# zkonduit/ezkl

Measured on AMD Instinct MI355X. Metric: BN254 G1 MSM pts/s (2^20 points per GPU; NTT 2^22 elems/s in extra), higher is better.
Workload: dtype u32x8 (254-bit modular integer, Montgomery); 1 GPU; configs[1]: standalone 2^20-point BN254 G1 MSM (uniform scalars, try-and-increment bases) + 2^22 scalar-field NTT per GPU; parallelism=points sharded across 1 rank(s); all_gather of 64-B partials + host fold

## Files before the change

ezkl_amd/csrc/msm.hip:

```cpp
#include "common.hpp"
#include <deque>
#include <thread>
#include <chrono>
#include "curve.hpp"
#include "curve29.hpp"
#include "host64.hpp"
#include <string.h>

namespace ezkl {

static constexpr uint32_t MSM_MAX_PART_BITS = 12;
static constexpr uint32_t MSM_SPAN_HEAVY = 16;
static constexpr uint32_t MSM_PART_STAGE = 13312;
static constexpr uint32_t MSM_BINSORT_STAGE = 15360;
static constexpr uint32_t MSM_HEAVY_CHUNK = 256;
static constexpr uint32_t MSM_DIGIT_E = 8;
static constexpr uint32_t MSM_LMIN = 8;
static constexpr uint32_t MSM_MAX_BIG = 64;
static constexpr uint32_t MSM_BIG_BLOCKS = 64;
static constexpr uint32_t MSM_BIG_ROWS = 8;

__device__ __forceinline__ uint32_t msm_part_of(uint32_t bucket, uint32_t NP) { return bucket ? 1u + (bucket & (NP - 1u)) : 0u; }
__device__ __forceinline__ uint32_t msm_lane_len(const uint32_t* offsets, uint32_t nb, uint32_t nlanes, uint32_t lmin) {
    const uint32_t l = (uint32_t)(((uint64_t)offsets[nb] + nlanes - 1) / nlanes);
    return l < lmin ? lmin : l;
}

template <class T> __device__ __forceinline__ T* bshift(T* p, size_t bytes) {
    return reinterpret_cast<T*>(reinterpret_cast<uintptr_t>(p) + bytes);
}
#define BSH(p) p = bshift(p, _bo)
#define BOFF() const size_t _bo = (size_t)blockIdx.z * bstride

struct WinPlan {
    uint32_t W, base, rem;
    __host__ __device__ uint32_t width(uint32_t w) const { return base + (w < rem ? 1u : 0u); }
    __host__ __device__ uint32_t offset(uint32_t w) const { return w * base + (w < rem ? w : rem); }
    __host__ __device__ uint32_t cmax() const { return base + (rem ? 1u : 0u); }
};
struct MsmTable {
    g1a_t* tab = nullptr;
    WinPlan wp{0, 0, 0};
    size_t n = 0;
    hipEvent_t ready = nullptr;
    bool synced = false;
};
struct MsmSlot;
struct MsmUpload;
struct MsmBatch;
struct MsmState;
static MsmState& msm_state();
#define g_tables (msm_state().tables)
#define g_table_stream (msm_state().table_stream)
#define g_slots (msm_state().slots)
#define g_call_slots (msm_state().call_slots)
#define g_call_claimed (msm_state().call_claimed)
#define g_call_finishing (msm_state().call_finishing)
#define g_call_owner (msm_state().call_owner)
#define g_call_order_ev (msm_state().call_order_ev)
#define g_copy_st (msm_state().copy_st)
#define g_tail_pinned (msm_state().tail_pinned)
#define g_tail_pinned_elems (msm_state().tail_pinned_elems)
#define g_open_upload (msm_state().open_upload)
#define g_open_batch (msm_state().open_batch)

static constexpr int MSM_MAX_SLOTS = 16;
static int msm_slots_init() {
    int v = 4;
    if (const char* e = getenv("EZKL_MSM_SLOTS")) {
        const int x = atoi(e);
        if (x >= 1 && x <= MSM_MAX_SLOTS) v = x;
    }
    return v;
}
static const int MSM_SLOTS = msm_slots_init();
struct MsmSlot {
    hipStream_t st = nullptr;
    uint8_t* scratch = nullptr;
    size_t scratch_bytes = 0;
    uint32_t* pinned = nullptr;
    void* pinned_dev = nullptr;
    size_t pinned_msms = 0;
    const fe_t** list_pinned = nullptr;
    hipEvent_t done = nullptr;
    uint32_t bits = 0;
    uint32_t count = 0;
    void* out = nullptr;
    bool busy = false;
};
static constexpr int MSM_CALL_SLOTS = 4;
struct MsmState {
    std::map<const Bases*, MsmTable> tables;
    hipStream_t table_stream = nullptr;
    MsmSlot slots[MSM_MAX_SLOTS];
    MsmSlot call_slots[MSM_CALL_SLOTS];
    bool call_claimed[MSM_CALL_SLOTS] = {false, false, false, false};
    bool call_finishing[MSM_CALL_SLOTS] = {false, false, false, false};
    std::thread::id call_owner[MSM_CALL_SLOTS];
    hipEvent_t call_order_ev = nullptr;
    hipStream_t copy_st = nullptr;
    fe_t* tail_pinned = nullptr;
    size_t tail_pinned_elems = 0;
    MsmUpload* open_upload = nullptr;
    MsmBatch* open_batch = nullptr;
    bool attrs_set = false;
    int acc_blocks_per_cu = 0;
};
static MsmState& msm_state() {
    Ctx* c = ctx();
    if (!c->msm_state) c->msm_state = new MsmState();
    return *static_cast<MsmState*>(c->msm_state);
}


static WinPlan pick_plan(size_t n) {
    WinPlan best{0, 0, 0};
    double best_cost = 0;
    for (uint32_t W = 10; W <= 127; W++) {
        WinPlan p{W, 254 / W, 254 % W};
        if (p.cmax() > 23) continue;
        const double cost = (double)n * W + 4.0 * (double)((size_t)1 << (p.cmax() - 1));
        if (!best.W || cost < best_cost) { best = p; best_cost = cost; }
    }
    return best;
}

__global__ __launch_bounds__(256) void msm_precompute_kernel(const g1a_t* prev, g1a_t* next, size_t n, uint32_t c) {
    size_t i = (size_t)blockIdx.x * blockDim.x + threadIdx.x;
    if (i >= n) return;
    g1a_t p = ld_g1a(prev + i);
    g1x_t a = g1x_from_affine(p);
    for (uint32_t k = 0; k < c; k++) a = g1x_double(a);
    st_g1a(next + i, g1x_to_affine(a));
}

__global__ __launch_bounds__(256) void msm_table_to_r261_kernel(g1a_t* tab, size_t count) {
    size_t i = (size_t)blockIdx.x * blockDim.x + threadIdx.x;
    if (i >= count) return;
    fe_t k;
#pragma unroll
    for (int q = 0; q < 8; q++) k.v[q] = Fq29C::R261_32[q];
    g1a_t p = ld_g1a(tab + i);
    if (g1a_is_id(p)) return;
    p.x = Fq::mul(p.x, k);
    p.y = Fq::mul(p.y, k);
    st_g1a(tab + i, p);
}

__device__ __forceinline__ bool gt_half_r(const fe_t& s) {
    uint32_t d[8], c = 0, br = 0;
#pragma unroll
    for (int i = 0; i < 8; i++) d[i] = addc32(s.v[i], s.v[i], c);
#pragma unroll
    for (int i = 0; i < 8; i++) (void)subb32(d[i], FrP::MOD[i], br);
    return c != 0 || br == 0;
}
__device__ __forceinline__ fe_t msm_canon(const fe_t* scalars, size_t i, uint32_t& neg) {
    fe_t s = Fr::from_mont(ld_fe(scalars + i));
    neg = 0;
    if (gt_half_r(s)) {
        uint32_t br = 0;
#pragma unroll
        for (int k = 0; k < 8; k++) s.v[k] = subb32(FrP::MOD[k], s.v[k], br);
        neg = 1;
    }
    return s;
}
__device__ __forceinline__ uint32_t msm_take_bits(fe_t& s, uint32_t c) {
    const uint32_t d = s.v[0] & ((1u << c) - 1u);
#pragma unroll
    for (int k = 0; k < 7; k++) s.v[k] = __builtin_amdgcn_alignbit(s.v[k + 1], s.v[k], c);
    s.v[7] >>= c;
    return d;
}
template <class F>
__device__ __forceinline__ void msm_foreach_digit(fe_t s, uint32_t neg, const WinPlan& wp, F&& f) {
    uint32_t carry = 0;
    for (uint32_t w = 0; w < wp.W; w++) {
        const uint32_t c = wp.width(w), half = 1u << (c - 1);
        uint32_t raw = msm_take_bits(s, c) + carry;
        if (raw > half) {
            carry = 1;
            if (raw != (1u << c)) f(w, (1u << c) - raw - 1u, neg ^ 1u);
        } else {
            carry = 0;
            if (raw) f(w, raw - 1u, neg);
        }
    }
}

__device__ __forceinline__ bool msm_digit_step(fe_t& s, uint32_t neg, uint32_t c, uint32_t& carry, uint32_t& bucket, uint32_t& sign) {
    const uint32_t half = 1u << (c - 1);
    const uint32_t raw = msm_take_bits(s, c) + carry;
    if (raw > half) {
        carry = 1;
        bucket = (1u << c) - raw - 1u;
        sign = neg ^ 1u;
        return raw != (1u << c);
    }
    carry = 0;
    bucket = raw - 1u;
    sign = neg;
    return raw != 0;
}

__device__ __forceinline__ uint32_t msm_block_scan(uint32_t v, uint32_t* wsum, uint32_t& total) {
    const uint32_t lane = threadIdx.x & 63u, wave = threadIdx.x >> 6, nw = blockDim.x >> 6;
    uint32_t x = v;
#pragma unroll
    for (uint32_t d = 1; d < 64; d <<= 1) {
        const uint32_t y = __shfl_up(x, d, 64);
        if (lane >= d) x += y;
    }
    if (lane == 63) wsum[wave] = x;
    __syncthreads();
    if (wave == 0) {
        uint32_t s = lane < nw ? wsum[lane] : 0u;
#pragma unroll
        for (uint32_t d = 1; d < 16; d <<= 1) {
            const uint32_t y = __shfl_up(s, d, 64);
            if (lane >= d) s += y;
        }
        if (lane < nw) wsum[lane] = s;
    }
    __syncthreads();
    total = wsum[nw - 1];
    const uint32_t r = x + (wave ? wsum[wave - 1] : 0u);
    __syncthreads();
    return r;
}

__global__ __launch_bounds__(256) void msm_hist_kernel(const fe_t* scalars, size_t n, size_t per_block, WinPlan wp,
                                                       uint32_t LB, uint32_t NP, uint32_t* wg_hist, uint32_t* wg_cnt,
                                                       const fe_t* const* scal_list, uint32_t* zero_base, uint32_t zero_words, size_t bstride) {
    BOFF(); BSH(wg_hist); BSH(wg_cnt);
    if (scal_list) scalars = scal_list[blockIdx.z];
    if (zero_base) {
        BSH(zero_base);
        for (uint32_t i = blockIdx.x * 256 + threadIdx.x; i < zero_words; i += gridDim.x * 256) zero_base[i] = 0;
    }
    __shared__ uint32_t lh[(1u << MSM_MAX_PART_BITS) + 1];
    const uint32_t NQ = NP + 1;
    for (uint32_t p = threadIdx.x; p < NQ; p += 256) lh[p] = 0;
    __syncthreads();
    size_t lo = (size_t)blockIdx.x * per_block, hi = lo + per_block < n ? lo + per_block : n;
    for (size_t i0 = lo + threadIdx.x; i0 < hi; i0 += 4 * 256) {
        fe_t s[4];
        uint32_t neg[4], carry[4] = {0, 0, 0, 0};
#pragma unroll
        for (int q = 0; q < 4; q++) {
            const size_t i = i0 + (size_t)q * 256;
            if (i < hi) s[q] = msm_canon(scalars, i, neg[q]);
            else { s[q] = Fr::zero(); neg[q] = 0; }
        }
        for (uint32_t w = 0; w < wp.W; w++) {
            const uint32_t c = wp.width(w);
#pragma unroll
            for (int q = 0; q < 4; q++) {
                uint32_t bucket, sign;
                if (msm_digit_step(s[q], neg[q], c, carry[q], bucket, sign)) atomicAdd(&lh[msm_part_of(bucket, NP)], 1u);
            }
        }
    }
    __syncthreads();
    for (uint32_t p = threadIdx.x; p < NQ; p += 256) {
        wg_hist[(size_t)blockIdx.x * NQ + p] = lh[p];
        wg_cnt[(size_t)blockIdx.x * NQ + p] = lh[p];
    }
}
__global__ __launch_bounds__(1024) void msm_hist_scan_kernel(uint32_t* wg_hist, uint32_t G, uint32_t NP, uint32_t* part_count, size_t bstride) {
    BOFF(); BSH(wg_hist); BSH(part_count);
    __shared__ uint32_t sums[32][33];
    const uint32_t c = threadIdx.x & 31, j = threadIdx.x >> 5;
    const uint32_t p = blockIdx.x * 32 + c;
    const uint32_t chunk = (G + 31) / 32, g0 = j * chunk, g1 = g0 + chunk < G ? g0 + chunk : G;
    uint32_t s = 0;
    if (p < NP)
        for (uint32_t g = g0; g < g1; g++) s += wg_hist[(size_t)g * NP + p];
    sums[j][c] = s;
    __syncthreads();
    if (j == 0) {
        uint32_t run = 0;
        for (uint32_t q = 0; q < 32; q++) {
            uint32_t v = sums[q][c];
            sums[q][c] = run;
            run += v;
        }
        if (p < NP) part_count[p] = run;
    }
    __syncthreads();
    if (p < NP) {
        uint32_t run = sums[j][c];
        for (uint32_t g = g0; g < g1; g++) {
            uint32_t v = wg_hist[(size_t)g * NP + p];
            wg_hist[(size_t)g * NP + p] = run;
            run += v;
        }
    }
}
__device__ __forceinline__ void msm_part_scan_body(const uint32_t* part_count, uint32_t NQ, uint32_t* part_base, uint32_t* big_flag,
                                                   uint32_t* big_list, uint32_t* big_count, uint32_t* sh) {
    const uint32_t t = threadIdx.x;
    constexpr uint32_t PER = 5;
    uint32_t v[PER], sum = 0;
#pragma unroll
    for (uint32_t q = 0; q < PER; q++) {
        const uint32_t i = PER * t + q;
        v[q] = i < NQ ? part_count[i] : 0;
        sum += v[q];
    }
    uint32_t total;
    uint32_t run = msm_block_scan(sum, sh, total) - sum;
#pragma unroll
    for (uint32_t q = 0; q < PER; q++) {
        const uint32_t i = PER * t + q;
        if (i < NQ) part_base[i] = run;
        run += v[q];
    }
    if (t == 1023) part_base[NQ] = total;
#pragma unroll
    for (uint32_t q = 0; q < PER; q++) {
        const uint32_t i = PER * t + q;
        if (i == 0 || i >= NQ) continue;
        uint32_t slot = 0;
        if (v[q] > MSM_BINSORT_STAGE) {
            slot = atomicAdd(big_count, 1u);
            if (slot < MSM_MAX_BIG) big_list[slot] = i - 1;
            slot = slot < MSM_MAX_BIG ? slot + 1 : 0;
        }
        big_flag[i - 1] = slot;
    }
}
__global__ __launch_bounds__(1024) void msm_part_scan_kernel(const uint32_t* part_count, uint32_t NQ, uint32_t* part_base, uint32_t* big_flag,
                                                             uint32_t* big_list, uint32_t* big_count, size_t bstride) {
    BOFF(); BSH(part_count); BSH(part_base); BSH(big_flag); BSH(big_list); BSH(big_count);
    __shared__ uint32_t sh[1024];
    msm_part_scan_body(part_count, NQ, part_base, big_flag, big_list, big_count, sh);
}
__global__ __launch_bounds__(1024) void msm_partition_kernel(const fe_t* scalars, size_t n, size_t per_block, WinPlan wp,
                                                             uint32_t LB, uint32_t NP, size_t base_offset, size_t tab_stride,
                                                             const uint32_t* part_base, const uint32_t* wg_hist, const uint32_t* wg_cnt, uint2* entries,
                                                             uint32_t* vals, const fe_t* const* scal_list, size_t bstride) {
    BOFF(); BSH(part_base); BSH(wg_hist); BSH(wg_cnt); BSH(entries); BSH(vals);
    if (scal_list) scalars = scal_list[blockIdx.z];
    extern __shared__ uint32_t plds[];
    __shared__ uint32_t tsum[1024];
    const uint32_t NQ = NP + 1;
    uint32_t* start = plds;
    uint32_t* cursor = plds + (NQ + 1);
    uint32_t* gbase = plds + 2 * (NQ + 1);
    uint2* stage = reinterpret_cast<uint2*>(plds + 3 * (NQ + 1));
    const uint32_t t = threadIdx.x, T = blockDim.x;
    const uint32_t K = (NQ + T - 1) / T;
    uint32_t loc = 0;
    for (uint32_t q = 0; q < K; q++) {
        const uint32_t p = t * K + q;
        if (p < NQ) loc += wg_cnt[(size_t)blockIdx.x * NQ + p];
    }
    uint32_t total;
    uint32_t run = msm_block_scan(loc, tsum, total) - loc;
    for (uint32_t q = 0; q < K; q++) {
        const uint32_t p = t * K + q;
        if (p < NQ) {
            start[p] = run;
            cursor[p] = run;
            gbase[p] = part_base[p] + wg_hist[(size_t)blockIdx.x * NQ + p];
            run += wg_cnt[(size_t)blockIdx.x * NQ + p];
        }
    }
    __syncthreads();
    const size_t lo = (size_t)blockIdx.x * per_block, hi = lo + per_block < n ? lo + per_block : n;
    const size_t i = lo + t;
    if (i < hi) {
        uint32_t neg;
        fe_t s = msm_canon(scalars, i, neg);
        msm_foreach_digit(s, neg, wp, [&](uint32_t w, uint32_t bucket, uint32_t sign) {
            const uint32_t r = atomicAdd(&cursor[msm_part_of(bucket, NP)], 1u);
            stage[r] = make_uint2((uint32_t)(w * tab_stride + base_offset + i) | (sign << 31), bucket);
        });
    }
    __syncthreads();
    const uint32_t PB = 31 - __clz(NP);
    for (uint32_t idx = t; idx < total; idx += T) {
        const uint2 e = stage[idx];
        const uint32_t p = msm_part_of(e.y, NP);
        const uint32_t slot = gbase[p] + (idx - start[p]);
        if (p) entries[slot] = make_uint2(e.x, e.y >> PB);
        else vals[slot] = e.x;
    }
}
__device__ __forceinline__ uint32_t msm_wave_rank(uint32_t* cnt, uint32_t key) {
    const uint64_t active = __ballot(1);
    const uint32_t first = __builtin_amdgcn_readfirstlane(key);
    if (__ballot(key == first) == active) {
        const uint32_t rank = (uint32_t)__popcll(active & ((1ull << (threadIdx.x & 63u)) - 1ull));
        uint32_t base = 0;
        if (rank == 0) base = atomicAdd(&cnt[first], (uint32_t)__popcll(active));
        return (uint32_t)__builtin_amdgcn_readfirstlane(base) + rank;
    }
    return atomicAdd(&cnt[key], 1u);
}
__device__ __forceinline__ void msm_bins_scan(uint32_t* cnt, uint32_t* tsum, uint32_t nbins, uint32_t p, uint32_t beg, const uint32_t* part_base,
                                              bool emit, uint32_t* offsets, g1x29_t* buckets) {
    const uint32_t t = threadIdx.x;
    uint32_t loc[4], s = 0;
#pragma unroll
    for (int q = 0; q < 4; q++) {
        uint32_t j = t * 4 + q;
        loc[q] = j < nbins ? cnt[j] : 0;
        s += loc[q];
    }
    uint32_t total;
    uint32_t run = msm_block_scan(s, tsum, total) - s;
#pragma unroll
    for (int q = 0; q < 4; q++) {
        uint32_t j = t * 4 + q;
        if (j < nbins) {
            cnt[j] = run;
            if (emit) {
                const bool b0 = (p == 0 && j == 0);
                offsets[(size_t)p * nbins + j] = b0 ? part_base[0] : beg + run;
                if (b0 ? part_base[1] == part_base[0] : loc[q] == 0) st_f29(&buckets[(size_t)p * nbins + j].zz, Fq29::zero());
            }
        }
        run += loc[q];
    }
    __syncthreads();
// ... 10 lines not shown
    __shared__ uint32_t tsum[512];
    extern __shared__ uint32_t stage[];
    if (blockIdx.x >= NP) {
        BSH(big_list); BSH(big_count); BSH(bin_total); BSH(block_off);
        const uint32_t w = blockIdx.x - NP;
        msm_bigsort_count_body(entries, part_base, LB, big_list, big_count, bin_total, block_off, cnt, w % MSM_BIG_BLOCKS, w / MSM_BIG_BLOCKS, MSM_BIG_ROWS);
        return;
    }
    const uint32_t p = blockIdx.x, t = threadIdx.x, nbins = 1u << LB;
    const uint32_t beg = part_base[p + 1], end = part_base[p + 2];
    if (p == NP - 1 && t == 0) offsets[(size_t)NP * nbins] = end;
    if (big_flag[p]) return;
    const bool staged = (end - beg) <= MSM_BINSORT_STAGE;
    for (uint32_t j = t; j < nbins; j += 512) cnt[j] = 0;
    __syncthreads();
    if (staged) {
        constexpr int PER = MSM_BINSORT_STAGE / 512;
        uint2 v[PER];
#pragma unroll
        for (int q = 0; q < PER; q++) {
            const uint32_t e = beg + t + (uint32_t)q * 512u;
            v[q] = e < end ? entries[e] : make_uint2(0u, 0xffffffffu);
        }
#pragma unroll
        for (int q = 0; q < PER; q++)
            if (v[q].y != 0xffffffffu) atomicAdd(&cnt[v[q].y], 1u);
        __syncthreads();
        msm_bins_scan(cnt, tsum, nbins, p, beg, part_base, true, offsets, buckets);
#pragma unroll
        for (int q = 0; q < PER; q++)
            if (v[q].y != 0xffffffffu) stage[atomicAdd(&cnt[v[q].y], 1u)] = v[q].x;
        __syncthreads();
        for (uint32_t i = t; i < end - beg; i += 512) vals[beg + i] = stage[i];
    } else {
        for (uint32_t e = beg + t; e < end; e += 512) (void)msm_wave_rank(cnt, entries[e].y);
        __syncthreads();
        msm_bins_scan(cnt, tsum, nbins, p, beg, part_base, true, offsets, buckets);
        for (uint32_t e = beg + t; e < end; e += 512) {
            const uint2 v = entries[e];
            vals[beg + msm_wave_rank(cnt, v.y)] = v.x;
        }
    }
}
__device__ __forceinline__ void msm_big_slice(uint32_t beg, uint32_t end, uint32_t& s0, uint32_t& s1, uint32_t bx) {
    const uint32_t chunk = (end - beg + MSM_BIG_BLOCKS - 1) / MSM_BIG_BLOCKS;
    s0 = beg + bx * chunk;
    s1 = s0 + chunk < end ? s0 + chunk : end;
    if (s0 > end) s0 = end;
}
__device__ __forceinline__ void msm_bigsort_count_body(const uint2* entries, const uint32_t* part_base, uint32_t LB, const uint32_t* big_list,
                                                       const uint32_t* big_count, uint32_t* bin_total, uint32_t* block_off, uint32_t* cnt, uint32_t bx,
                                                       uint32_t by, uint32_t rows) {
    const uint32_t t = threadIdx.x, nbins = 1u << LB;
    const uint32_t nbig = big_count[0] < MSM_MAX_BIG ? big_count[0] : MSM_MAX_BIG;
    for (uint32_t y = by; y < nbig; y += rows) {
        const uint32_t p = big_list[y];
        uint32_t s0, s1;
        msm_big_slice(part_base[p + 1], part_base[p + 2], s0, s1, bx);
        for (uint32_t j = t; j < nbins; j += 512) cnt[j] = 0;
        __syncthreads();
        for (uint32_t e = s0 + t; e < s1; e += 512) (void)msm_wave_rank(cnt, entries[e].y);
        __syncthreads();
        for (uint32_t j = t; j < nbins; j += 512)
            block_off[((size_t)y * MSM_BIG_BLOCKS + bx) * nbins + j] = cnt[j] ? atomicAdd(&bin_total[(size_t)y * nbins + j], cnt[j]) : 0u;
        __syncthreads();
    }
}
__global__ __launch_bounds__(512) void msm_bigsort_scatter_kernel(const uint2* entries, const uint32_t* part_base, uint32_t LB, const uint32_t* big_list,
                                                                  const uint32_t* big_count, const uint32_t* bin_total, const uint32_t* block_off,
                                                                  uint32_t* offsets, uint32_t* vals, g1x29_t* buckets, size_t bstride) {
    BOFF(); BSH(entries); BSH(part_base); BSH(big_list); BSH(big_count); BSH(bin_total); BSH(block_off); BSH(offsets); BSH(vals); BSH(buckets);
    __shared__ uint32_t cnt[2048];
    __shared__ uint32_t tsum[512];
    const uint32_t t = threadIdx.x, nbins = 1u << LB;
    const uint32_t nbig = big_count[0] < MSM_MAX_BIG ? big_count[0] : MSM_MAX_BIG;
    for (uint32_t y = blockIdx.y; y < nbig; y += gridDim.y) {
        const uint32_t p = big_list[y], beg = part_base[p + 1];
        uint32_t s0, s1;
        msm_big_slice(beg, part_base[p + 2], s0, s1, blockIdx.x);
        for (uint32_t j = t; j < nbins; j += 512) cnt[j] = bin_total[(size_t)y * nbins + j];
        __syncthreads();
        msm_bins_scan(cnt, tsum, nbins, p, beg, part_base, blockIdx.x == 0, offsets, buckets);
        const uint32_t* mine = block_off + ((size_t)y * MSM_BIG_BLOCKS + blockIdx.x) * nbins;
        for (uint32_t j = t; j < nbins; j += 512) cnt[j] += mine[j];
        __syncthreads();
        for (uint32_t e = s0 + t; e < s1; e += 512) {
            const uint2 v = entries[e];
            vals[beg + msm_wave_rank(cnt, v.y)] = v.x;
        }
        __syncthreads();
    }
}

struct MsmRec {
    g1a_t p;
    bool neg;
};
__device__ __forceinline__ MsmRec msm_fetch(const g1a_t* tab, uint32_t v) {
    MsmRec r;
    r.p = ld_g1a(tab + (v & 0x7fffffffu));
    r.neg = (v >> 31) != 0;
    return r;
}
__global__ __launch_bounds__(256, 3) void msm_accumulate_kernel(const g1a_t* tab, const uint32_t* offsets, const uint32_t* vals,
                                                             uint32_t nb, uint32_t nlanes, g1x29_t* buckets, g1x29_t* head, g1x29_t* tail,
                                                             uint32_t* lane_first, uint32_t lmin, size_t bstride) {
    BOFF(); BSH(offsets); BSH(vals); BSH(buckets); BSH(head); BSH(tail); BSH(lane_first);
    const uint32_t t = blockIdx.x * blockDim.x + threadIdx.x;
    const uint32_t total = offsets[nb], L = msm_lane_len(offsets, nb, nlanes, lmin);
    const uint64_t k0w = (uint64_t)t * L;
    if (k0w >= total) return;
    const uint32_t k0 = (uint32_t)k0w;
    const uint32_t k1 = (uint64_t)k0 + L < total ? k0 + L : total;
    uint32_t lo = 0, hi = nb;
    while (hi - lo > 1) {
        uint32_t mid = (lo + hi) >> 1;
        if (offsets[mid] <= k0) lo = mid; else hi = mid;
    }
    uint32_t b = lo, bin_end = offsets[b + 1];
    uint32_t end_next = offsets[b + 2 <= nb ? b + 2 : nb];
    lane_first[t] = b;
    bool started_before = offsets[b] < k0;
    g1x29_t acc = g1x29_identity();
    MsmRec nxt = msm_fetch(tab, vals[k0]);
    uint32_t vn = k0 + 1 < k1 ? vals[k0 + 1] : 0u;
    for (uint32_t k = k0; k < k1; k++) {
        if (k == bin_end) {
            if (started_before) st_g1x29(head + t, acc); else st_g1x29(buckets + b, acc);
            acc.zz = Fq29::zero();
            started_before = false;
            b++;
            bin_end = end_next;
            if (bin_end == k) {
                uint32_t probes = 1;
                while (bin_end == k && probes < 4) { b++; bin_end = offsets[b + 1]; probes++; }
                if (bin_end == k) {
                    uint32_t lo2 = b + 1, hi2 = nb;
                    while (hi2 - lo2 > 1) {
                        uint32_t mid = (lo2 + hi2) >> 1;
                        if (offsets[mid] <= k) lo2 = mid; else hi2 = mid;
                    }
                    b = lo2;
                    bin_end = offsets[b + 1];
                }
            }
            end_next = offsets[b + 2 <= nb ? b + 2 : nb];
        }
        const MsmRec cur = nxt;
        nxt = msm_fetch(tab, vn);
        vn = k + 2 < k1 ? vals[k + 2] : 0u;
        acc = g1x29_add_mixed(acc, g1a29_unpack(cur.p), cur.neg);
    }
    if (k1 == bin_end) {
        if (started_before) st_g1x29(head + t, acc); else st_g1x29(buckets + b, acc);
    } else {
        if (started_before) st_g1x29(head + t, acc); else st_g1x29(tail + t, acc);
    }
}
EZ_D g1x29_t g1x29_shfl_down(const g1x29_t& p, uint32_t d) {
    g1x29_t r;
    const uint32_t* s = p.x.v;
    uint32_t* o = r.x.v;
#pragma unroll
    for (int k = 0; k < 36; k++) o[k] = __shfl_down(s[k], d);
    return r;
}
__global__ __launch_bounds__(256) void msm_fixup_boundary_tree_kernel(const uint32_t* offsets, uint32_t nb, uint32_t nlanes,
                                                                      const uint32_t* lane_first, const g1x29_t* head, const g1x29_t* tail, g1x29_t* buckets,
                                                                      uint32_t* heavy_list, uint32_t* heavy_count, uint32_t* chunk_list, uint32_t lmin,
                                                                      uint32_t span_heavy, size_t bstride) {
    BOFF(); BSH(offsets); BSH(lane_first); BSH(head); BSH(tail); BSH(buckets); BSH(heavy_list); BSH(heavy_count); BSH(chunk_list);
    const uint32_t t = blockIdx.x * blockDim.x + threadIdx.x + 1;
    const uint32_t lane = threadIdx.x & 63u;
    const uint32_t L = msm_lane_len(offsets, nb, nlanes, lmin);
    const uint64_t k0 = (uint64_t)t * L;
    bool cut = t < nlanes && k0 < offsets[nb];
    uint32_t b = 0, t1 = 0, t2 = 0;
    if (cut) {
        b = lane_first[t];
        const uint32_t beg = offsets[b], end = offsets[b + 1];
        cut = beg < k0;
        t1 = beg / L; t2 = (end - 1) / L;
    }
    if (cut && t2 - t1 > span_heavy) {
        if (t == t1 + 1 && t2 - t1 > MSM_HEAVY_CHUNK) heavy_list[atomicAdd(heavy_count, 1u)] = b;
        if ((t - t1 - 1) % MSM_HEAVY_CHUNK == 0) chunk_list[atomicAdd(heavy_count + 1, 1u)] = t;
        cut = false;
    }
    const uint32_t wave_last = t + (63u - lane);
    const uint32_t run = cut ? (t2 < wave_last ? t2 : wave_last) - t + 1u : 0u;
    uint32_t longest = run;
#pragma unroll
    for (uint32_t o = 32; o > 0; o >>= 1) {
        const uint32_t m = __shfl_xor(longest, o);
        longest = m > longest ? m : longest;
    }
    if (longest == 0) return;
    if (longest <= 2) {
        if (!cut || t != t1 + 1) return;
        g1x29_t acc = g1x29_add(ld_g1x29(tail + t1), ld_g1x29(head + t));
        for (uint32_t u = t + 1; u <= t2; u++) acc = g1x29_add(acc, ld_g1x29(head + u));
        st_g1x29(buckets + b, acc);
        return;
    }
    g1x29_t v = cut ? ld_g1x29(head + t) : g1x29_identity();
    uint32_t have = cut ? 1u : 0u;
#pragma unroll 1
    for (uint32_t d = 1; d < longest; d <<= 1) {
        const g1x29_t w = g1x29_shfl_down(v, d);
        const uint32_t hw = __shfl_down(have, d);
        if (have == d && run > d) {
            v = g1x29_add(v, w);
            have += hw;
        }
    }
    if (!cut || t != t1 + 1) return;
    g1x29_t acc = g1x29_add(ld_g1x29(tail + t1), v);
    for (uint32_t u = t + run; u <= t2; u++) acc = g1x29_add(acc, ld_g1x29(head + u));
    st_g1x29(buckets + b, acc);
}
__global__ __launch_bounds__(256) void msm_fixup_heavy1_kernel(const uint32_t* offsets, uint32_t nb, uint32_t nlanes, const uint32_t* lane_first, g1x29_t* head,
                                                               const g1x29_t* tail, g1x29_t* buckets, const uint32_t* chunk_list, const uint32_t* counts, uint32_t lmin,
                                                               uint32_t coop, size_t bstride) {
    BOFF(); BSH(offsets); BSH(lane_first); BSH(head); BSH(tail); BSH(buckets); BSH(chunk_list); BSH(counts);
    const uint32_t nchunks = counts[1], L = msm_lane_len(offsets, nb, nlanes, lmin);
    const uint32_t wave = threadIdx.x >> 6, lane = threadIdx.x & 63u;
    for (uint32_t ci = blockIdx.x * 4u + wave; ci < nchunks; ci += gridDim.x * 4u) {
        const uint32_t start = chunk_list[ci], b = lane_first[start];
        const uint32_t t2 = (offsets[b + 1] - 1) / L;
        const uint32_t stop = start + MSM_HEAVY_CHUNK - 1 < t2 ? start + MSM_HEAVY_CHUNK - 1 : t2;
        const uint32_t t1 = offsets[b] / L;
        const bool whole = t2 - t1 <= MSM_HEAVY_CHUNK;
        g1x29_t acc = (whole && lane == 63u) ? ld_g1x29(tail + t1) : g1x29_identity();
        for (uint32_t t = start + lane; t <= stop; t += 64) acc = g1x29_add(acc, ld_g1x29(head + t));
        acc = coop ? g1x29_group_sum_coop(acc, 64) : g1x29_group_sum(acc, 64);
        if (lane == 0) st_g1x29(whole ? buckets + b : head + start, acc);
    }
}
__global__ __launch_bounds__(256) void msm_fixup_heavy2_kernel(const uint32_t* offsets, uint32_t nb, uint32_t nlanes, const g1x29_t* head, const g1x29_t* tail,
                                                               const uint32_t* heavy_list, const uint32_t* counts, g1x29_t* buckets, uint32_t lmin, uint32_t coop, size_t bstride) {
    BOFF(); BSH(offsets); BSH(head); BSH(tail); BSH(heavy_list); BSH(counts); BSH(buckets);
    const uint32_t L = msm_lane_len(offsets, nb, nlanes, lmin);
    const uint32_t wave = threadIdx.x >> 6, lane = threadIdx.x & 63u;
    for (uint32_t h = blockIdx.x * 4u + wave; h < counts[0]; h += gridDim.x * 4u) {
        const uint32_t b = heavy_list[h];
        const uint32_t t1 = offsets[b] / L, t2 = (offsets[b + 1] - 1) / L;
        g1x29_t acc = lane == 63u ? ld_g1x29(tail + t1) : g1x29_identity();
        for (uint32_t t = t1 + 1 + lane * MSM_HEAVY_CHUNK; t <= t2; t += 64 * MSM_HEAVY_CHUNK) acc = g1x29_add(acc, ld_g1x29(head + t));
        acc = coop ? g1x29_group_sum_coop(acc, 64) : g1x29_group_sum(acc, 64);
        if (lane == 0) st_g1x29(buckets + b, acc);
// ... 37 lines not shown
    acc = (coop && lanes >= 4) ? g1x29_group_sum_coop(acc, lanes) : g1x29_group_sum(acc, lanes);
    if (j == 0 && o < nout) st_g1x29((isA ? SA : T) + o, acc);
}
__global__ __launch_bounds__(256) void msm_planes_kernel(const g1x29_t* SA, const g1x29_t* T, ReduceGeom g, g1x29_t* planes, g1x29_t* planes_host, uint32_t coop,
                                                         size_t bstride) {
    BOFF(); BSH(SA); BSH(T); BSH(planes);
    __shared__ uint4 sh[9 * 4];
    uint32_t id = blockIdx.x, field = 0, j = 0;
    if (id > 0) {
        id -= 1;
        if (id < g.wA) { field = 1; j = id; }
        else if (id < g.wA + g.wB) { field = 2; j = id - g.wA; }
        else { field = 3; j = id - g.wA - g.wB; }
    }
    const uint32_t nA = 1u << g.wA, nT = 1u << (g.wB + g.wC);
    g1x29_t acc = g1x29_identity();
    auto with_bit = [](uint32_t k, uint32_t bit) { return ((k >> bit) << (bit + 1)) | (1u << bit) | (k & ((1u << bit) - 1u)); };
    if (field == 0) {
        for (uint32_t d = threadIdx.x; d < nA; d += 256) acc = g1x29_add(acc, ld_g1x29(SA + d));
    } else if (field == 1) {
        for (uint32_t k = threadIdx.x; k < nA / 2; k += 256) acc = g1x29_add(acc, ld_g1x29(SA + with_bit(k, j)));
    } else {
        const uint32_t sh_bits = field == 2 ? j : g.wB + j;
        for (uint32_t k = threadIdx.x; k < nT / 2; k += 256) acc = g1x29_add(acc, ld_g1x29(T + with_bit(k, sh_bits)));
    }
    acc = (coop & 8u) ? g1x29_block256_sum_coop_full(acc, sh) : coop ? g1x29_block256_sum_coop(acc, sh) : g1x29_block256_sum(acc, sh);
    if (threadIdx.x == 0) {
        const uint32_t ws = field == 1 ? g.wsA : field == 2 ? g.wsB : g.wsC;
        const uint32_t slot = field == 0 ? 0u : 1u + ws + j;
        st_g1x29(planes + slot, acc);
        if (planes_host) st_g1x29(planes_host + (size_t)blockIdx.z * 32 + slot, acc);
    }
}

static int table_build(Ctx* c, hipStream_t st, const Bases* b, bool wait) {
    MsmTable t;
    t.n = b->n;
    t.wp = pick_plan(b->n);
    if ((size_t)t.wp.W * t.n >= ((size_t)1 << 31)) return EZKL_ERR_UNSUPPORTED;
    EZ_HIP(hipMalloc(&t.tab, (size_t)t.wp.W * t.n * sizeof(g1a_t)));
    EZ_HIP(hipMemcpyAsync(t.tab, b->pts, t.n * sizeof(g1a_t), hipMemcpyDeviceToDevice, st));
    for (uint32_t w = 1; w < t.wp.W; w++)
        hipLaunchKernelGGL(msm_precompute_kernel, dim3(cdiv(t.n, 256)), dim3(256), 0, st, t.tab + (size_t)(w - 1) * t.n,
                           t.tab + (size_t)w * t.n, t.n, t.wp.width(w - 1));
    hipLaunchKernelGGL(msm_table_to_r261_kernel, dim3(cdiv((size_t)t.wp.W * t.n, 256)), dim3(256), 0, st, t.tab, (size_t)t.wp.W * t.n);
    EZ_HIP(hipGetLastError());
    EZ_HIP(hipEventCreateWithFlags(&t.ready, hipEventDisableTiming));
    EZ_HIP(hipEventRecord(t.ready, st));
    if (wait) {
        EZ_HIP(hipStreamSynchronize(st));
        t.synced = true;
    }
    g_tables[b] = t;
    return EZKL_OK;
}
static int table_get(Ctx* c, hipStream_t st, const Bases* b, MsmTable** out) {
    auto it = g_tables.find(b);
    if (it == g_tables.end()) {
        int rc = table_build(c, st, b, true);
        if (rc) return rc;
        it = g_tables.find(b);
    }
    if (!it->second.synced) {
        EZ_HIP(hipEventSynchronize(it->second.ready));
        it->second.synced = true;
    }
    *out = &it->second;
    return EZKL_OK;
}
int msm_table_prepare(Ctx* c, const Bases* b) {
    if (g_tables.count(b)) return EZKL_OK;
    if (!g_table_stream) EZ_HIP(hipStreamCreateWithFlags(&g_table_stream, hipStreamNonBlocking));
    return table_build(c, g_table_stream, b, false);
}
void msm_table_drop(const Bases* b) {
    auto it = g_tables.find(b);
    if (it != g_tables.end()) {
        if (it->second.ready) { (void)hipEventSynchronize(it->second.ready); (void)hipEventDestroy(it->second.ready); }
        (void)hipFree(it->second.tab);
        g_tables.erase(it);
    }
}

static constexpr size_t MSM_MAX_GROUP = 16;
static int slot_prepare(MsmSlot& sl, size_t bytes, size_t msms = 1) {
    if (!sl.st) {
        EZ_HIP(stream_create_prio(&sl.st, "EZKL_HIP_PRIO_MSM", 0));
        EZ_HIP(hipEventCreateWithFlags(&sl.done, hipEventDisableTiming));
        EZ_HIP(hipHostMalloc((void**)&sl.list_pinned, MSM_MAX_GROUP * sizeof(void*), hipHostMallocDefault));
    }
    if (msms > sl.pinned_msms) {
        if (sl.pinned) {
            EZ_HIP(hipStreamSynchronize(sl.st));
            EZ_HIP(hipHostFree(sl.pinned));
            sl.pinned = nullptr;
        }
        EZ_HIP(hipHostMalloc((void**)&sl.pinned, msms * 32 * sizeof(g1x29_t), hipHostMallocDefault));
        EZ_HIP(hipHostGetDevicePointer(&sl.pinned_dev, sl.pinned, 0));
        sl.pinned_msms = msms;
    }
    if (bytes > sl.scratch_bytes) {
        if (sl.scratch) {
            EZ_HIP(hipStreamSynchronize(sl.st));
            EZ_HIP(hipFree(sl.scratch));
            sl.scratch = nullptr;
            sl.scratch_bytes = 0;
        }
        size_t want = bytes + (bytes >> 4);
        EZ_HIP(hipMalloc((void**)&sl.scratch, want));
        sl.scratch_bytes = want;
    }
    return EZKL_OK;
}
static int msm_finish(MsmSlot& sl, void* out_host = nullptr, bool release = true) {
    if (!out_host) out_host = sl.out;
    EZ_HIP(hipEventSynchronize(sl.done));
    for (uint32_t j = 0; j < sl.count; j++) {
        const uint32_t* hp = sl.pinned + (size_t)j * 32 * 36;
        h64::xyzz acc = h64::identity();
        for (int k = (int)sl.bits - 1; k >= 0; k--) {
            acc = h64::dbl(acc);
            acc = h64::add(acc, h64::from_limbs29_point(hp + 36 * (1 + k)));
        }
        acc = h64::add(acc, h64::from_limbs29_point(hp));
        h64::aff r = h64::to_affine(acc);
        memcpy((uint8_t*)out_host + 64 * (size_t)j, &r, 64);
    }
    if (release) sl.busy = false;
    return EZKL_OK;
}

static size_t msm_group_size(const MsmTable* T, size_t n, bool small_scalars, size_t batch = 0) {
    if (const char* e = getenv("EZKL_MSM_GROUP")) {
        const int v = atoi(e);
        if (v >= 1 && v <= (int)MSM_MAX_GROUP) return (size_t)v;
    }
    (void)T; (void)n; (void)batch;
    if (small_scalars) {
        static const int small = [] { const char* e = getenv("EZKL_MSM_GROUP_SMALL"); const int v = e ? atoi(e) : 0; return v >= 1 && v <= (int)MSM_MAX_GROUP ? v : 6; }();
        return (size_t)small;
    }
    static const int big = [] { const char* e = getenv("EZKL_MSM_GROUP_BIG"); const int v = e ? atoi(e) : 0; return v >= 1 && v <= (int)MSM_MAX_GROUP ? v : 4; }();
    return (size_t)big;
}
static int msm_enqueue(Ctx* c, MsmSlot& sl, hipStream_t st, MsmTable* T, size_t base_offset, const fe_t* const* cols, size_t count, size_t n, bool timed) {
    int rc = EZKL_OK;
    if (count < 1 || count > MSM_MAX_GROUP) return EZKL_ERR_INVALID;
    const unsigned Z = (unsigned)count;
    const fe_t* scalars = cols[0];
    const WinPlan wp = T->wp;
    const uint32_t W = wp.W, bits = wp.cmax() - 1;
    const uint32_t nb = 1u << bits;
    const size_t npairs = n * W;
    uint32_t PB = bits < 10 ? bits : 10;
    while (PB < bits && PB < MSM_MAX_PART_BITS && (npairs >> PB) > (size_t)MSM_BINSORT_STAGE * 9 / 10) PB++;
    const uint32_t LB = bits - PB, NP = 1u << PB;
    int& acc_blocks_per_cu = msm_state().acc_blocks_per_cu;
    if (!acc_blocks_per_cu) {
        EZ_HIP(hipFuncSetAttribute((const void*)msm_binsort_kernel, hipFuncAttributeMaxDynamicSharedMemorySize, 96 * 1024));
        EZ_HIP(hipFuncSetAttribute((const void*)msm_partition_kernel, hipFuncAttributeMaxDynamicSharedMemorySize, 144 * 1024));
        EZ_HIP(hipOccupancyMaxActiveBlocksPerMultiprocessor(&acc_blocks_per_cu, msm_accumulate_kernel, 256, 0));
        if (acc_blocks_per_cu < 1) acc_blocks_per_cu = 1;
    }
    const size_t resident = (size_t)acc_blocks_per_cu * 256 * c->num_cus;
    const size_t load = npairs >> bits, per_lane = load * 9 / 10 > 40 ? load * 9 / 10 : 40;
    size_t rounds = npairs / (resident * per_lane);
    if (rounds < 1) rounds = 1;
    uint32_t L = (uint32_t)((npairs + resident * rounds - 1) / (resident * rounds));
    if (L < 8) L = 8;
    if (const char* e = getenv("EZKL_MSM_L")) {
        const int v = atoi(e);
        if (v > 0 && v < (1 << 20)) L = (uint32_t)v;
    }
    const uint32_t nlanes = cdiv(npairs, L);
    static const uint32_t lmin = [] { const char* e = getenv("EZKL_MSM_LMIN"); const int v = e ? atoi(e) : 0; return (uint32_t)(v >= 1 && v <= 4096 ? v : (int)MSM_LMIN); }();
    constexpr uint32_t coop = 7;
    static const uint32_t span_heavy = [] { const char* e = getenv("EZKL_MSM_SPAN"); const int v = e ? atoi(e) : 0; return (uint32_t)(v >= 1 && v <= 4096 ? v : (int)MSM_SPAN_HEAVY); }();
    ReduceGeom rg;
    memset(&rg, 0, sizeof rg);
    if (LB > 0) {
        rg.wA = LB; rg.wsA = PB;
        rg.wB = (PB + 1) / 2; rg.wsB = 0;
        rg.wC = PB - rg.wB; rg.wsC = rg.wB;
    } else {
        rg.wA = (bits + 2) / 3; rg.wsA = 0;
        rg.wB = (bits - rg.wA + 1) / 2; rg.wsB = rg.wA;
        rg.wC = bits - rg.wA - rg.wB; rg.wsC = rg.wA + rg.wB;
    }
    {
        const uint32_t rows = 1u << (rg.wB + rg.wC), cols = 1u << rg.wA;
        uint32_t E = MSM_DIGIT_E;
        if (const char* e = getenv("EZKL_MSM_E")) {
            const int v = atoi(e);
            if (v > 0 && v <= 1024 && (v & (v - 1)) == 0) E = (uint32_t)v;
        }
        rg.EA = rows < E ? rows : E; rg.GA = rows / rg.EA;
        rg.ET = cols < E ? cols : E; rg.GT = cols / rg.ET;
    }
    const uint32_t nA = 1u << rg.wA, nT = 1u << (rg.wB + rg.wC);
    const uint32_t n_partA = nA * rg.GA, n_partT = nT * rg.GT;
    const uint32_t nplanes = 1 + bits;
    size_t per_block = MSM_PART_STAGE / W / 64 * 64;
    {
        const size_t lds_words = (144u << 10) / 4, fixed = 3 * ((size_t)NP + 2);
        const size_t fit = lds_words > fixed ? (lds_words - fixed) / (2 * (size_t)W) / 64 * 64 : 64;
        if (per_block > fit) per_block = fit;
    }
    if (per_block > 1024) per_block = 1024;
    if (per_block < 64) per_block = 64;
    const unsigned sgrid = cdiv(n, per_block);
    auto al = [](size_t x) { return (x + 255) & ~(size_t)255; };
    size_t off = 0;
    auto carve = [&](size_t bytes) { size_t o = off; off += al(bytes); return o; };
    size_t o_list = carve(MSM_MAX_GROUP * sizeof(void*));
    size_t o_ent = carve(npairs * 8), o_vals = carve(npairs * 4), o_offs = carve(((size_t)nb + 1) * 4);
    const uint32_t NQ = NP + 1;
    size_t o_pcnt = carve((NQ + 1) * 4), o_pbase = carve((NQ + 1) * 4), o_wgh = carve((size_t)sgrid * NQ * 4), o_wgc = carve((size_t)sgrid * NQ * 4);
    size_t o_heavy = carve((size_t)nb * 4), o_chunks = carve(((size_t)nlanes + 1) * 4);
    const size_t nbins = (size_t)1 << LB;
    size_t o_hcnt = carve(256), o_btot = carve(MSM_MAX_BIG * nbins * 4), o_planes = carve((size_t)nplanes * sizeof(g1x29_t));
    const size_t zero_bytes = off - o_hcnt;
    size_t o_bflag = carve((size_t)NP * 4), o_blist = carve(MSM_MAX_BIG * 4),
           o_boff = carve((size_t)MSM_MAX_BIG * MSM_BIG_BLOCKS * nbins * 4);
    size_t o_lfirst = carve((size_t)nlanes * 4);
    size_t o_bkt = carve((size_t)nb * sizeof(g1x29_t));
    size_t o_head = carve((size_t)nlanes * sizeof(g1x29_t)), o_tail = carve((size_t)nlanes * sizeof(g1x29_t));
    size_t o_partA = carve((size_t)n_partA * sizeof(g1x29_t)), o_partT = carve((size_t)n_partT * sizeof(g1x29_t));
    size_t o_SA = carve((size_t)nA * sizeof(g1x29_t)), o_T = carve((size_t)nT * sizeof(g1x29_t));
    const size_t bstride = count > 1 ? off : 0;
    rc = slot_prepare(sl, off * count, count);
    if (rc) return rc;
    uint8_t* S = sl.scratch;
    const fe_t* const* scal_list = nullptr;
    if (count > 1) {
        for (size_t j = 0; j < count; j++) sl.list_pinned[j] = cols[j];
        EZ_HIP(hipMemcpyAsync(S + o_list, sl.list_pinned, count * sizeof(void*), hipMemcpyHostToDevice, st));
        scal_list = (const fe_t* const*)(S + o_list);
    }
    uint2* entries = (uint2*)(S + o_ent);
    uint32_t* vals = (uint32_t*)(S + o_vals);
    uint32_t* offs = (uint32_t*)(S + o_offs);
    uint32_t *pcnt = (uint32_t*)(S + o_pcnt), *pbase = (uint32_t*)(S + o_pbase), *wghist = (uint32_t*)(S + o_wgh), *wgcnt = (uint32_t*)(S + o_wgc);
    uint32_t *heavy = (uint32_t*)(S + o_heavy), *hcnt = (uint32_t*)(S + o_hcnt), *chunks = (uint32_t*)(S + o_chunks);
    uint32_t* lfirst = (uint32_t*)(S + o_lfirst);
    uint32_t *bflag = (uint32_t*)(S + o_bflag), *blist = (uint32_t*)(S + o_blist), *btot = (uint32_t*)(S + o_btot), *boff = (uint32_t*)(S + o_boff);
    uint32_t* bcnt = hcnt + 2;
    g1x29_t *bkt = (g1x29_t*)(S + o_bkt), *head = (g1x29_t*)(S + o_head), *tail = (g1x29_t*)(S + o_tail);
    g1x29_t *partA = (g1x29_t*)(S + o_partA), *partT = (g1x29_t*)(S + o_partT), *SA = (g1x29_t*)(S + o_SA), *TT = (g1x29_t*)(S + o_T);
    g1x29_t* planes = (g1x29_t*)(S + o_planes);

    hipEvent_t m0 = nullptr, m1 = nullptr, a0 = nullptr, a1 = nullptr;
    bool timed_chain = timed;
    if (timed) {
        const char* tm = getenv("EZKL_HIP_TIMING");
        if (tm && !strcmp(tm, "none")) timed = timed_chain = false;
        else if (tm && !strcmp(tm, "kernel")) timed_chain = false;
    }
    if (timed) {
        if (timed_chain && (rc = ev_pair(c, "msm", &m0, &m1))) return rc;
        if ((rc = ev_pair(c, "msm_accumulate", &a0, &a1))) return rc;
        if (timed_chain) EZ_HIP(hipEventRecord(m0, st));
    }
    hipLaunchKernelGGL(msm_hist_kernel, dim3(sgrid, 1, Z), dim3(256), 0, st, scalars, n, per_block, wp, LB, NP, wghist, wgcnt, scal_list, hcnt,
                       (uint32_t)(zero_bytes / 4), bstride);
    hipLaunchKernelGGL(msm_hist_scan_kernel, dim3(cdiv(NQ, 32), 1, Z), dim3(1024), 0, st, wghist, sgrid, NQ, pcnt, bstride);
    hipLaunchKernelGGL(msm_part_scan_kernel, dim3(1, 1, Z), dim3(1024), 0, st, pcnt, NQ, pbase, bflag, blist, bcnt, bstride);
    hipLaunchKernelGGL(msm_partition_kernel, dim3(sgrid, 1, Z), dim3((unsigned)per_block), (3 * ((size_t)NQ + 1) + 2 * per_block * W) * 4, st, scalars, n, per_block, wp,
                       LB, NP, base_offset, T->n, pbase, wghist, wgcnt, entries, vals, scal_list, bstride);
    hipLaunchKernelGGL(msm_binsort_kernel, dim3(NP + MSM_BIG_BLOCKS * MSM_BIG_ROWS, 1, Z), dim3(512), MSM_BINSORT_STAGE * 4, st, entries, pbase, LB, NP, bflag, offs,
                       vals, bkt, blist, bcnt, btot, boff, bstride);
    hipLaunchKernelGGL(msm_bigsort_scatter_kernel, dim3(MSM_BIG_BLOCKS, MSM_BIG_ROWS, Z), dim3(512), 0, st, entries, pbase, LB, blist, bcnt, btot, boff, offs,
                       vals, bkt, bstride);
    if (timed) EZ_HIP(hipEventRecord(a0, st));
    hipLaunchKernelGGL(msm_accumulate_kernel, dim3(cdiv(nlanes, 256), 1, Z), dim3(256), 0, st, T->tab, offs, vals, nb, nlanes, bkt, head, tail,
                       lfirst, lmin, bstride);
    if (timed) EZ_HIP(hipEventRecord(a1, st));
    if (nlanes > 1)
    {
        hipLaunchKernelGGL(msm_fixup_boundary_tree_kernel, dim3(cdiv(nlanes - 1, 256), 1, Z), dim3(256), 0, st, offs, nb, nlanes, lfirst, head, tail, bkt,
                           heavy, hcnt, chunks, lmin, span_heavy, bstride);
    }
    {
        size_t max_heavy = nlanes / span_heavy + 1;
        const size_t heavy_wgs = (max_heavy + 3) / 4;
        unsigned hb = (unsigned)(heavy_wgs < (size_t)c->num_cus * 4 ? heavy_wgs : (size_t)c->num_cus * 4);
        size_t max_chunks = nlanes / MSM_HEAVY_CHUNK + max_heavy;
        const size_t chunk_wgs = (max_chunks + 3) / 4;
        unsigned cb = (unsigned)(chunk_wgs < (size_t)c->num_cus * 4 ? chunk_wgs : (size_t)c->num_cus * 4);
        hipLaunchKernelGGL(msm_fixup_heavy1_kernel, dim3(cb, 1, Z), dim3(256), 0, st, offs, nb, nlanes, lfirst, head, tail, bkt, chunks, hcnt, lmin, coop & 4u, bstride);
        hipLaunchKernelGGL(msm_fixup_heavy2_kernel, dim3(hb, 1, Z), dim3(256), 0, st, offs, nb, nlanes, head, tail, heavy, hcnt, bkt, lmin, coop & 4u, bstride);
    }
    {
        const uint32_t th = n_partA > n_partT ? n_partA : n_partT;
        hipLaunchKernelGGL(msm_reduce1_kernel, dim3(cdiv(th, 256), 2, Z), dim3(256), 0, st, bkt, rg, partA, partT, bstride);
        auto pow2_le = [](uint32_t x) { uint32_t p = 1; while (p * 2 <= x) p *= 2; return p; };
        uint32_t lanesA = pow2_le(rg.GA < 64 ? rg.GA : 64), lanesT = pow2_le(rg.GT < 64 ? rg.GT : 64);
        auto waves = [&](uint32_t nout, uint32_t lanes) { return cdiv(nout, 64 / lanes); };
        while (waves(nA, lanesA) + waves(nT, lanesT) > (unsigned)c->num_cus * 4 && (lanesA > 1 || lanesT > 1)) {
            if (lanesT > 1 && waves(nT, lanesT) >= waves(nA, lanesA)) lanesT >>= 1; else if (lanesA > 1) lanesA >>= 1; else lanesT >>= 1;
        }
        const uint32_t blocksA = waves(nA, lanesA);
        hipLaunchKernelGGL(msm_reduce2_kernel, dim3(blocksA + waves(nT, lanesT), 1, Z), dim3(64), 0, st, partA, partT, rg, SA, TT, lanesA, lanesT, blocksA, coop & 1u, bstride);
        hipLaunchKernelGGL(msm_planes_kernel, dim3(nplanes, 1, Z), dim3(256), 0, st, SA, TT, rg, planes, (g1x29_t*)sl.pinned_dev,
                           coop & 10u, bstride);
    }
    EZ_HIP(hipGetLastError());
    if (getenv("EZKL_MSM_DEBUG")) {
        uint32_t hc = 0;
        EZ_HIP(hipMemcpyAsync(&hc, hcnt, 4, hipMemcpyDeviceToHost, st));
        EZ_HIP(hipStreamSynchronize(st));
        fprintf(stderr, "[msm] n=%zu W=%u bits=%u L=%u nlanes=%u heavy=%u\n", n, W, bits, L, nlanes, hc);
    }
    if (timed_chain) EZ_HIP(hipEventRecord(m1, st));
    EZ_HIP(hipEventRecord(sl.done, st));
    sl.bits = bits;
    sl.count = (uint32_t)count;
    sl.busy = true;
    return EZKL_OK;
}
static int msm_run_groups(Ctx* c, MsmTable* T, size_t base_offset, const fe_t* const* cols, size_t batch, size_t n, void* out_host,
                          const hipEvent_t* wait_ev, bool small_scalars) {
    const size_t G = msm_group_size(T, n, small_scalars, batch);
    static const bool dbg = getenv("EZKL_MSM_DEBUG") != nullptr;
    if (dbg) fprintf(stderr, "[ezkl_hip] msm batch: %zu columns of %zu points, %s scalars, groups of %zu\n", batch, n, small_scalars ? "witness-shaped" : "general", G);
    int rc = EZKL_OK;
    size_t gi = 0;
    for (size_t j0 = 0; j0 < batch && !rc; gi++) {
        size_t cnt = batch - j0 < G ? batch - j0 : G;
        if (wait_ev && j0 > 0) {
            const size_t left = batch - j0;
            cnt = left <= 2 ? 1 : std::min(G, (left + 1) / 2);
        }
        MsmSlot& sl = g_slots[gi % MSM_SLOTS];
        if (sl.busy) rc = msm_finish(sl);
        if (!rc) rc = slot_prepare(sl, 0);
        for (size_t j = 0; wait_ev && j < cnt && !rc; j++)
            if (hipStreamWaitEvent(sl.st, wait_ev[j0 + j], 0) != hipSuccess) rc = EZKL_ERR_HIP;
        if (!rc) {
            sl.out = (uint8_t*)out_host + 64 * j0;
            rc = msm_enqueue(c, sl, sl.st, T, base_offset, cols + j0, cnt, n, false);
        }
        j0 += cnt;
    }
    for (size_t k = 0; k < (size_t)MSM_SLOTS; k++) {
        MsmSlot& sl = g_slots[(gi + k) % MSM_SLOTS];
        if (!sl.busy) continue;
        if (!rc) rc = msm_finish(sl);
        else { (void)hipStreamSynchronize(sl.st); sl.busy = false; }
    }
    return rc;
}
// ... 464 lines not shown
```

Measured before the change: 800.1 million pts/s.

## Pass scalar column pointers by value and tweak binsort, accumulate and fixup kernels

Scalar column pointers now go to the hist and partition kernels inside a by-value struct kernel argument, which removes the pinned host list and its host-to-device copy for grouped MSMs. The bigsort count merge now uses shared-memory atomics. The accumulate kernel's binary search reuses the upper-bound value it already loaded, and its next-offset load moves out of the branch. The fixup kernel gets an occupancy hint in its launch bounds. For the single-MSM benchmark, the per-launch host work changes little, and the atomics and launch-bound changes may shift register use or contention.

```diff
diff --git a/ezkl_amd/csrc/msm.hip b/ezkl_amd/csrc/msm.hip
--- a/ezkl_amd/csrc/msm.hip
+++ b/ezkl_amd/csrc/msm.hip
@@ -26,11 +26,17 @@
     return l < lmin ? lmin : l;
 }
 
-template <class T> __device__ __forceinline__ T* bshift(T* p, size_t bytes) {
-    return reinterpret_cast<T*>(reinterpret_cast<uintptr_t>(p) + bytes);
+template <class T> __device__ __forceinline__ T* bshift(T* p, size_t bytes) { return reinterpret_cast<T*>(reinterpret_cast<char*>(p) + bytes); }
+template <class T> __device__ __forceinline__ const T* bshift(const T* p, size_t bytes) {
+    return reinterpret_cast<const T*>(reinterpret_cast<const char*>(p) + bytes);
 }
 #define BSH(p) p = bshift(p, _bo)
 #define BOFF() const size_t _bo = (size_t)blockIdx.z * bstride
+static constexpr size_t MSM_MAX_GROUP = 16;
+struct MsmCols {
+    const fe_t* col[MSM_MAX_GROUP];
+};
+__device__ __forceinline__ const fe_t* msm_col(const MsmCols& cols) { return cols.col[blockIdx.z]; }
 
 struct WinPlan {
     uint32_t W, base, rem;
@@ -81,7 +87,6 @@
     uint32_t* pinned = nullptr;
     void* pinned_dev = nullptr;
     size_t pinned_msms = 0;
-    const fe_t** list_pinned = nullptr;
     hipEvent_t done = nullptr;
     uint32_t bits = 0;
     uint32_t count = 0;
@@ -230,11 +235,11 @@
     return r;
 }
 
-__global__ __launch_bounds__(256) void msm_hist_kernel(const fe_t* scalars, size_t n, size_t per_block, WinPlan wp,
+__global__ __launch_bounds__(256) void msm_hist_kernel(MsmCols cols, size_t n, size_t per_block, WinPlan wp,
                                                        uint32_t LB, uint32_t NP, uint32_t* wg_hist, uint32_t* wg_cnt,
-                                                       const fe_t* const* scal_list, uint32_t* zero_base, uint32_t zero_words, size_t bstride) {
+                                                       uint32_t* zero_base, uint32_t zero_words, size_t bstride) {
     BOFF(); BSH(wg_hist); BSH(wg_cnt);
-    if (scal_list) scalars = scal_list[blockIdx.z];
+    const fe_t* scalars = msm_col(cols);
     if (zero_base) {
         BSH(zero_base);
         for (uint32_t i = blockIdx.x * 256 + threadIdx.x; i < zero_words; i += gridDim.x * 256) zero_base[i] = 0;
@@ -337,12 +342,12 @@
     __shared__ uint32_t sh[1024];
     msm_part_scan_body(part_count, NQ, part_base, big_flag, big_list, big_count, sh);
 }
-__global__ __launch_bounds__(1024) void msm_partition_kernel(const fe_t* scalars, size_t n, size_t per_block, WinPlan wp,
+__global__ __launch_bounds__(1024) void msm_partition_kernel(MsmCols cols, size_t n, size_t per_block, WinPlan wp,
                                                              uint32_t LB, uint32_t NP, size_t base_offset, size_t tab_stride,
                                                              const uint32_t* part_base, const uint32_t* wg_hist, const uint32_t* wg_cnt, uint2* entries,
-                                                             uint32_t* vals, const fe_t* const* scal_list, size_t bstride) {
+                                                             uint32_t* vals, size_t bstride) {
     BOFF(); BSH(part_base); BSH(wg_hist); BSH(wg_cnt); BSH(entries); BSH(vals);
-    if (scal_list) scalars = scal_list[blockIdx.z];
+    const fe_t* scalars = msm_col(cols);
     extern __shared__ uint32_t plds[];
     __shared__ uint32_t tsum[1024];
     const uint32_t NQ = NP + 1;
@@ -519,7 +524,7 @@
         __syncthreads();
         msm_bins_scan(cnt, tsum, nbins, p, beg, part_base, blockIdx.x == 0, offsets, buckets);
         const uint32_t* mine = block_off + ((size_t)y * MSM_BIG_BLOCKS + blockIdx.x) * nbins;
-        for (uint32_t j = t; j < nbins; j += 512) cnt[j] += mine[j];
+        for (uint32_t j = t; j < nbins; j += 512) atomicAdd(&cnt[j], mine[j]);
         __syncthreads();
         for (uint32_t e = s0 + t; e < s1; e += 512) {
             const uint2 v = entries[e];
@@ -572,17 +577,17 @@
                 uint32_t probes = 1;
                 while (bin_end == k && probes < 4) { b++; bin_end = offsets[b + 1]; probes++; }
                 if (bin_end == k) {
-                    uint32_t lo2 = b + 1, hi2 = nb;
+                    uint32_t lo2 = b + 1, hi2 = nb, vhi = total;
                     while (hi2 - lo2 > 1) {
-                        uint32_t mid = (lo2 + hi2) >> 1;
-                        if (offsets[mid] <= k) lo2 = mid; else hi2 = mid;
+                        const uint32_t mid = (lo2 + hi2) >> 1, vm = offsets[mid];
+                        if (vm <= k) lo2 = mid; else { hi2 = mid; vhi = vm; }
                     }
                     b = lo2;
-                    bin_end = offsets[b + 1];
+                    bin_end = vhi;
                 }
             }
-            end_next = offsets[b + 2 <= nb ? b + 2 : nb];
-        }
+        }
+        end_next = offsets[b + 2 <= nb ? b + 2 : nb];
         const MsmRec cur = nxt;
         nxt = msm_fetch(tab, vn);
         vn = k + 2 < k1 ? vals[k + 2] : 0u;
@@ -602,7 +607,7 @@
     for (int k = 0; k < 36; k++) o[k] = __shfl_down(s[k], d);
     return r;
 }
-__global__ __launch_bounds__(256) void msm_fixup_boundary_tree_kernel(const uint32_t* offsets, uint32_t nb, uint32_t nlanes,
+__global__ __launch_bounds__(256, 3) void msm_fixup_boundary_tree_kernel(const uint32_t* offsets, uint32_t nb, uint32_t nlanes,
                                                                       const uint32_t* lane_first, const g1x29_t* head, const g1x29_t* tail, g1x29_t* buckets,
                                                                       uint32_t* heavy_list, uint32_t* heavy_count, uint32_t* chunk_list, uint32_t lmin,
                                                                       uint32_t span_heavy, size_t bstride) {
@@ -806,12 +811,10 @@
     }
 }
 
-static constexpr size_t MSM_MAX_GROUP = 16;
 static int slot_prepare(MsmSlot& sl, size_t bytes, size_t msms = 1) {
     if (!sl.st) {
         EZ_HIP(stream_create_prio(&sl.st, "EZKL_HIP_PRIO_MSM", 0));
         EZ_HIP(hipEventCreateWithFlags(&sl.done, hipEventDisableTiming));
-        EZ_HIP(hipHostMalloc((void**)&sl.list_pinned, MSM_MAX_GROUP * sizeof(void*), hipHostMallocDefault));
     }
     if (msms > sl.pinned_msms) {
         if (sl.pinned) {
@@ -871,7 +874,6 @@
     int rc = EZKL_OK;
     if (count < 1 || count > MSM_MAX_GROUP) return EZKL_ERR_INVALID;
     const unsigned Z = (unsigned)count;
-    const fe_t* scalars = cols[0];
     const WinPlan wp = T->wp;
     const uint32_t W = wp.W, bits = wp.cmax() - 1;
     const uint32_t nb = 1u << bits;
@@ -936,7 +938,6 @@
     auto al = [](size_t x) { return (x + 255) & ~(size_t)255; };
     size_t off = 0;
     auto carve = [&](size_t bytes) { size_t o = off; off += al(bytes); return o; };
-    size_t o_list = carve(MSM_MAX_GROUP * sizeof(void*));
     size_t o_ent = carve(npairs * 8), o_vals = carve(npairs * 4), o_offs = carve(((size_t)nb + 1) * 4);
     const uint32_t NQ = NP + 1;
     size_t o_pcnt = carve((NQ + 1) * 4), o_pbase = carve((NQ + 1) * 4), o_wgh = carve((size_t)sgrid * NQ * 4), o_wgc = carve((size_t)sgrid * NQ * 4);
@@ -955,12 +956,8 @@
     rc = slot_prepare(sl, off * count, count);
     if (rc) return rc;
     uint8_t* S = sl.scratch;
-    const fe_t* const* scal_list = nullptr;
-    if (count > 1) {
-        for (size_t j = 0; j < count; j++) sl.list_pinned[j] = cols[j];
-        EZ_HIP(hipMemcpyAsync(S + o_list, sl.list_pinned, count * sizeof(void*), hipMemcpyHostToDevice, st));
-        scal_list = (const fe_t* const*)(S + o_list);
-    }
+    MsmCols kcols;
+    for (size_t j = 0; j < MSM_MAX_GROUP; j++) kcols.col[j] = cols[j < count ? j : 0];
     uint2* entries = (uint2*)(S + o_ent);
     uint32_t* vals = (uint32_t*)(S + o_vals);
     uint32_t* offs = (uint32_t*)(S + o_offs);
@@ -985,12 +982,12 @@
         if ((rc = ev_pair(c, "msm_accumulate", &a0, &a1))) return rc;
         if (timed_chain) EZ_HIP(hipEventRecord(m0, st));
     }
-    hipLaunchKernelGGL(msm_hist_kernel, dim3(sgrid, 1, Z), dim3(256), 0, st, scalars, n, per_block, wp, LB, NP, wghist, wgcnt, scal_list, hcnt,
+    hipLaunchKernelGGL(msm_hist_kernel, dim3(sgrid, 1, Z), dim3(256), 0, st, kcols, n, per_block, wp, LB, NP, wghist, wgcnt, hcnt,
                        (uint32_t)(zero_bytes / 4), bstride);
     hipLaunchKernelGGL(msm_hist_scan_kernel, dim3(cdiv(NQ, 32), 1, Z), dim3(1024), 0, st, wghist, sgrid, NQ, pcnt, bstride);
     hipLaunchKernelGGL(msm_part_scan_kernel, dim3(1, 1, Z), dim3(1024), 0, st, pcnt, NQ, pbase, bflag, blist, bcnt, bstride);
-    hipLaunchKernelGGL(msm_partition_kernel, dim3(sgrid, 1, Z), dim3((unsigned)per_block), (3 * ((size_t)NQ + 1) + 2 * per_block * W) * 4, st, scalars, n, per_block, wp,
-                       LB, NP, base_offset, T->n, pbase, wghist, wgcnt, entries, vals, scal_list, bstride);
+    hipLaunchKernelGGL(msm_partition_kernel, dim3(sgrid, 1, Z), dim3((unsigned)per_block), (3 * ((size_t)NQ + 1) + 2 * per_block * W) * 4, st, kcols, n, per_block, wp,
+                       LB, NP, base_offset, T->n, pbase, wghist, wgcnt, entries, vals, bstride);
     hipLaunchKernelGGL(msm_binsort_kernel, dim3(NP + MSM_BIG_BLOCKS * MSM_BIG_ROWS, 1, Z), dim3(512), MSM_BINSORT_STAGE * 4, st, entries, pbase, LB, NP, bflag, offs,
                        vals, bkt, blist, bcnt, btot, boff, bstride);
     hipLaunchKernelGGL(msm_bigsort_scatter_kernel, dim3(MSM_BIG_BLOCKS, MSM_BIG_ROWS, Z), dim3(512), 0, st, entries, pbase, LB, blist, bcnt, btot, boff, offs,
```

Result: faster. 811.4 million pts/s, median of 6 (+1.4%).
